# PorousMediaSimulation/openLBMPM

Hardware: AMD Instinct MI355X
Metric: MLUPS (million lattice updates/s) (higher is better)
Workload: dtype f64

## Files before the change

openlbmpm_amd/csrc/rk3dq.h:

```cpp

constexpr int QS = 23;
constexpr unsigned CELLB = QS * 8u;
constexpr int QLINE = 16;
constexpr int SR = 12, SC = 68;
constexpr int SCOMP = SR * SC;
constexpr int SSLOT = 4 * SCOMP;

typedef const unsigned long long __attribute__((address_space(4))) *const_u64_ptr;
__device__ __forceinline__ unsigned long long pstart_of(const RK3Dev &p, int zl) { return ((const_u64_ptr)p.pstart)[zl]; }

struct PlaneAddrQ {
    const char *base;
    unsigned off[3], cnt[3];
};

__device__ __forceinline__ PlaneAddrQ plane_addr_q(const RK3Dev &p, const double *f, int zl)
{
    PlaneAddrQ a;
    const unsigned long long p1 = pstart_of(p, zl), p2 = pstart_of(p, zl + 1);
    const unsigned long long p0 = zl > 0 ? pstart_of(p, zl - 1) : p1, p3 = zl <= p.nzl ? pstart_of(p, zl + 2) : p2;
    a.base = reinterpret_cast<const char *>(f) + (size_t)p0 * CELLB;
    a.cnt[0] = (unsigned)(p1 - p0); a.cnt[1] = (unsigned)(p2 - p1); a.cnt[2] = (unsigned)(p3 - p2);
    a.off[0] = 0u; a.off[1] = a.cnt[0] * CELLB; a.off[2] = a.off[1] + a.cnt[1] * CELLB;
    return a;
}

template <bool ASM>
__device__ __forceinline__ double ldq(const char *uniform_base, unsigned off)
{
    if (!ASM) return ldg(uniform_base, off);
    double v;
    asm volatile("global_load_dwordx2 %0, %1, %2" : "=v"(v) : "v"(off), "s"(uniform_base));
    return v;
}
#define LBMPM_WAIT_VMCNT0 0x0F70

template <bool FIRST, bool UNI, typename Rows, bool ASM = false>
__device__ __forceinline__ void pull_q(const RK3Dev &p, const Rows &rows, int zl, unsigned b, double g[Q], unsigned &own_j)
{
    constexpr int OPP[Q] = LBMPM_D3Q19_OPP;
    const PlaneAddrQ a = plane_addr_q(p, p.fin, zl);
    {
        const RowTab t = rows(zl, 0);
        own_j = t.first + bits_below<UNI>(t.m, b);
    }
    const unsigned own8 = own_j * 8u;
    if (FIRST) {
#pragma unroll
        for (int i = 0; i < Q; ++i) g[i] = ldq<ASM>(a.base, a.off[1] + (unsigned)i * a.cnt[1] * 8u + own8);
        return;
    }
#pragma unroll
    for (int rz = -1; rz <= 1; ++rz)
#pragma unroll
        for (int ry = -1; ry <= 1; ++ry) {
            const RowTab t = rows(zl + rz, ry);
#pragma unroll
            for (int dx = -1; dx <= 1; ++dx) {
                const int i = DIRT[(1 - rz) * 9 + (1 - ry) * 3 + (1 - dx)];
                if (i < 0) continue;
                unsigned off;
                if (i == 0) off = a.off[1] + own8;
                else {
                    unsigned j;
                    bool fl;
                    row_cell<UNI>(t, dx, b, j, fl);
                    const unsigned up = a.off[1 + rz] + (unsigned)i * a.cnt[1 + rz] * 8u + j * 8u;
                    const unsigned back = a.off[1] + (unsigned)OPP[i] * a.cnt[1] * 8u + own8;
                    off = fl ? up : back;
                }
                g[i] = ldq<ASM>(a.base, off);
            }
        }
}

__device__ __forceinline__ unsigned row_index(const RK3Dev &p, int zl, int y, int sg) { return ((unsigned)zl * (unsigned)p.ny + (unsigned)y) * (unsigned)p.nseg + (unsigned)sg; }

struct LdsScal {
    const double *tile;
    int own;
    int slot[3];
    typedef int H;
    __device__ __forceinline__ H own_cell() const { return slot[1] + own; }
    __device__ __forceinline__ H cell(int rz, int ry, int dx, bool fl, unsigned, unsigned, unsigned) const { return fl ? slot[1 + rz] + own + ry * SC + dx : slot[1] + own; }
    __device__ __forceinline__ double comp(H h, int k) const { return tile[h + k * SCOMP]; }
};
struct GlbScal {
    const uint32_t *pur_in;
    int ny, nseg;
    const char *base;
    unsigned soff[3];
    unsigned own_j;
    int zp, sg, y;
    struct H { unsigned off, cst; };
    __device__ __forceinline__ H at(int rz, int ry, int sgs, unsigned j) const
    {
        int s = sg + sgs;
        s = s < 0 ? s + nseg : (s >= nseg ? s - nseg : s);
        H h;
        h.cst = pur_in[((size_t)(zp + rz) * ny + wrapi(y + ry, ny)) * nseg + s];
        h.off = soff[1 + rz] + j * 32u;
        return h;
    }
    __device__ __forceinline__ H own_cell() const { return at(0, 0, 0, own_j); }
    __device__ __forceinline__ H cell(int rz, int ry, int dx, bool fl, unsigned j, unsigned b, unsigned last) const
    {
        if (!fl) return own_cell();
        return at(rz, ry, (dx < 0 && b == 0u) ? -1 : ((dx > 0 && b == last) ? 1 : 0), j);
    }
    __device__ __forceinline__ double comp(H h, int k) const
    {
        if (h.cst) return k == 0 && (h.cst & 1u) ? 1. : 0.;
        return *reinterpret_cast<const double *>(base + h.off + 8u * (unsigned)k);
    }
};
__device__ __forceinline__ GlbScal glb_scal(const RK3Dev &p, const PlaneAddrQ &a, unsigned own_j, int zp, int sg, int y)
{
    GlbScal s{p.pur_in, p.ny, p.nseg, a.base, {0u, 0u, 0u}, own_j, zp, sg, y};
#pragma unroll
    for (int k = 0; k < 3; ++k) s.soff[k] = a.off[k] + (unsigned)Q * a.cnt[k] * 8u;
    return s;
}

struct Sums { double k0, kp, km, a0, ap, am, t0, tp, tm; };

template <int CLS, bool FIRST, bool UNI, typename Rows, typename Scal>
__device__ __forceinline__ void class_sum_one(const RK3Dev &p, const Rows &rows, const Scal &sc, int zp, unsigned b, const double g[Q],
                                              double &ks, double &as, double &ts)
{
#pragma clang fp contract(off)
    constexpr int CX[Q] = LBMPM_D3Q19_CX, CY[Q] = LBMPM_D3Q19_CY, CZ[Q] = LBMPM_D3Q19_CZ;
    constexpr int rz = -CLS;
    ks = 0.; as = 0.; ts = 0.;
    if (CLS == 0) { ks = sc.comp(sc.own_cell(), 0) * g[0]; ts = g[0]; }
#pragma unroll
    for (int ry = -1; ry <= 1; ++ry) {
        RowTab t{};
        if (!FIRST) t = rows(zp + rz, ry);
#pragma unroll
        for (int dx = -1; dx <= 1; ++dx) {
            const int i = DIRT[(1 - rz) * 9 + (1 - ry) * 3 + (1 - dx)];
            if (i <= 0) continue;
            unsigned j = 0;
            bool fl = true;
            typename Scal::H h;
            if (FIRST) h = sc.own_cell();
            else {
                row_cell<UNI>(t, dx, b, j, fl);
                h = sc.cell(rz, ry, dx, fl, j, b, t.last);
            }
            const double k = sc.comp(h, 0);
            double ea = 0.;
            bool any = false;
            if (CX[i] != 0) { const double v = sc.comp(h, 1); ea = CX[i] > 0 ? v : -v; any = true; }
            if (CY[i] != 0) { const double v = sc.comp(h, 2); ea = any ? (CY[i] > 0 ? ea + v : ea - v) : (CY[i] > 0 ? v : -v); any = true; }
            if (CZ[i] != 0) { const double v = sc.comp(h, 3); ea = any ? (CZ[i] > 0 ? ea + v : ea - v) : (CZ[i] > 0 ? v : -v); }
            const double c = i < 7 ? p.rcA : p.rcD;
            const double cs = fl ? c : -c;
            ks = __builtin_fma(k, g[i], ks); as = __builtin_fma(cs, ea, as); ts += g[i];
        }
    }
}

template <bool FIRST, bool UNI, typename Rows, typename Scal>
__device__ __forceinline__ void class_sums(const RK3Dev &p, const Rows &rows, const Scal &sc, int zp, unsigned b, const double g[Q], Sums &S)
{
    class_sum_one<1, FIRST, UNI>(p, rows, sc, zp, b, g, S.kp, S.ap, S.tp);
    class_sum_one<0, FIRST, UNI>(p, rows, sc, zp, b, g, S.k0, S.a0, S.t0);
    class_sum_one<-1, FIRST, UNI>(p, rows, sc, zp, b, g, S.km, S.am, S.tm);
}

template <int CLS, bool FIRST, typename Rows>
__device__ __forceinline__ void pull_class(const RK3Dev &p, const Rows &rows, int zl, unsigned b, unsigned own_j, double g[Q])
{
    constexpr int OPP[Q] = LBMPM_D3Q19_OPP;
    constexpr int rz = -CLS;
    const PlaneAddrQ a = plane_addr_q(p, p.fin, zl);
    const unsigned own8 = own_j * 8u;
    if (CLS == 0) g[0] = ldg(a.base, a.off[1] + own8);
#pragma unroll
    for (int ry = -1; ry <= 1; ++ry) {
        RowTab t{};
        if (!FIRST) t = rows(zl + rz, ry);
#pragma unroll
        for (int dx = -1; dx <= 1; ++dx) {
            const int i = DIRT[(1 - rz) * 9 + (1 - ry) * 3 + (1 - dx)];
            if (i <= 0) continue;
            unsigned j = 0;
            bool fl = true;
            if (!FIRST) row_cell<false>(t, dx, b, j, fl);
            const unsigned up = a.off[1 + rz] + (unsigned)i * a.cnt[1 + rz] * 8u + j * 8u;
            const unsigned back = a.off[1] + (unsigned)OPP[i] * a.cnt[1] * 8u + own8;
            g[i] = ldg(a.base, FIRST ? a.off[1] + (unsigned)i * a.cnt[1] * 8u + own8 : (fl ? up : back));
        }
    }
}

__device__ __forceinline__ void class_sums_pure(const double g[Q], bool red, Sums &S)
{
#pragma clang fp contract(off)
    constexpr int CZ[Q] = LBMPM_D3Q19_CZ;
    S.t0 = g[0]; S.tp = 0.; S.tm = 0.;
#pragma unroll
    for (int rz = -1; rz <= 1; ++rz)
#pragma unroll
        for (int ry = -1; ry <= 1; ++ry)
#pragma unroll
            for (int dx = -1; dx <= 1; ++dx) {
                const int i = DIRT[(1 - rz) * 9 + (1 - ry) * 3 + (1 - dx)];
                if (i <= 0) continue;
                if (CZ[i] == 0) S.t0 += g[i];
                else if (CZ[i] > 0) S.tp += g[i];
                else S.tm += g[i];
            }
    S.k0 = red ? S.t0 : 0.; S.kp = red ? S.tp : 0.; S.km = red ? S.tm : 0.;
    S.a0 = S.ap = S.am = 0.;
}

template <bool WITH_G, int PIN = -1>
__device__ __forceinline__ void bc_q(const RK3Dev &p, int zl, const Sums &S, double *g, double &rR, double &rho)
{
#pragma clang fp contract(off)
    const bool pin = PIN < 0 ? p.inletP != 0 : PIN == 1;
    const int zsg = p.z0 + source_plane(p, zl) - 1;
    const double r0 = S.k0 + S.a0, rp = S.kp + S.ap, rm = S.km + S.am;
    rR = (r0 + rp) + rm;
    rho = (S.t0 + S.tp) + S.tm;
    if (zsg == p.nzg - 2) {
        const double wR = r0 + 2. * rp, wT = S.t0 + 2. * S.tp;
        double J;
        if (pin) {
            rR = p.vzR;
            rho = p.vzR + p.vzB;
            J = wT - rho;
        } else {
            const double dR = wR / (1. + p.vzR), dB = (wT - wR) / (1. + p.vzB);
            rR = dR;
            rho = dR + dB;
            J = dR * p.vzR + dB * p.vzB;
        }
        if (WITH_G) {
            const double Nx = 0.5 * ((g[1] + g[7] + g[9]) - (g[2] + g[8] + g[10]));
            const double Ny = 0.5 * ((g[3] + g[7] + g[10]) - (g[4] + g[8] + g[9]));
            g[6] = g[5] - 1. / 3. * J;
            g[12] = g[11] - 1. / 6. * J + Nx;
            g[13] = g[14] - 1. / 6. * J - Nx;
            g[16] = g[15] - 1. / 6. * J + Ny;
            g[17] = g[18] - 1. / 6. * J - Ny;
        }
    }
    if (zsg == 1) {
        rR = p.rhoOutR;
        rho = p.rhoOutR + p.rhoOutB;
        if (WITH_G) {
            const double J = rho - (S.t0 + 2. * S.tm);
            const double Nx = 0.5 * ((g[1] + g[7] + g[9]) - (g[2] + g[8] + g[10]));
            const double Ny = 0.5 * ((g[3] + g[7] + g[10]) - (g[4] + g[8] + g[9]));
            g[5] = g[6] + 1. / 3. * J;
            g[11] = g[12] + 1. / 6. * J - Nx;
            g[14] = g[13] + 1. / 6. * J + Nx;
            g[15] = g[16] + 1. / 6. * J - Ny;
            g[18] = g[17] + 1. / 6. * J + Ny;
        }
    }
}
__device__ __forceinline__ double phi_q(double rR, double rho) { return (rR - (rho - rR)) / rho; }

template <bool FIRST, bool MRT, bool RAGGED, bool PIN = false>
__global__ __launch_bounds__(512, 1) void rk3dq_fused(RK3Dev p, int tilesX, int tilesY, int rows_per_xcd, int chunk_len, int z_first, int z_last,
                                                       int nchunks1, int z_first2, int z_last2,
                                                       unsigned *slotq)
{
    constexpr int TX = 64, TY = 8;
    using M = March<TX, TY>;
    using TR = TileRows<TY>;
    constexpr int CX[Q] = LBMPM_D3Q19_CX, CY[Q] = LBMPM_D3Q19_CY, CZ[Q] = LBMPM_D3Q19_CZ;
    __shared__ double sphi[M::RING][M::FY][M::FX];
    __shared__ double ssc[4 * SSLOT];
    __shared__ u32x4 srow[TR::SLOTS][TR::ROWS][6];
    __shared__ int sslot[2];
    const int tid = threadIdx.x;
    const int band_slots = (int)(gridDim.x >> 3);
    if (tid == 0 && !slotq) { sslot[0] = (int)(blockIdx.x & 7u); sslot[1] = (int)(blockIdx.x >> 3); }
    if (tid == 0 && slotq) {
        const int here = (int)(__builtin_amdgcn_s_getreg((3 << 11) | 20) & 7u);
        int band = -1, slot = 0;
        for (int k = 0; k < 8 && band < 0; ++k) {
            const int b = (here + k) & 7;
            const int q = (int)atomicAdd(&slotq[b], 1u);
            if (q < band_slots) { band = b; slot = q; }
        }
        sslot[0] = band; sslot[1] = slot;
    }
    __syncthreads();
    const int xcd = sslot[0], slot = sslot[1];
    if (xcd < 0) return;
#ifdef LBMPM_DEV
    const int bid = xcd + 8 * slot;
#endif
    const int tx = slot % tilesX, r = slot / tilesX, ty = xcd * rows_per_xcd + r % rows_per_xcd, chunk = r / rows_per_xcd;
    if (ty >= tilesY) return;
    const int wave = __builtin_amdgcn_readfirstlane(tid >> 6);
#ifdef LBMPM_DEV
    unsigned long long *trace = p.trace && z_last - z_first >= 8 ? p.trace + (size_t)bid * 4 : nullptr;
    if (trace && tid == 0) trace[0] = wall_clock64();
#endif
    int lx, ly, x, y, yo, hlx, hly, hx, hy, xrow, xc, xcol;
    bool own, has_own, has_rim, has_x, row_ok;
    TileRowsU<TY, true, RAGGED> rows_own{{srow, 0, 1}}, rows_rimrow{{srow, 0, 1}}, rows_xrow{{srow, 0, 1}};
    TileRowsU<TY, false, RAGGED> rows_rimcol{{srow, 0, 0}}, rows_xcol{{srow, 0, 0}};
    const int x0 = RAGGED ? seg_x0(tx, p.nx, tilesX) : tx * TX;
    const int tw = RAGGED ? seg_x0(tx + 1, p.nx, tilesX) - x0 : TX;
    const int twl = RAGGED ? (tx > 0 ? x0 - seg_x0(tx - 1, p.nx, tilesX) : p.nx - seg_x0(tilesX - 1, p.nx, tilesX)) : TX;
    auto set_geometry = [&](int t) {
        lx = t % TX; ly = t / TX;
        x = x0 + lx; y = ty * TY + ly;
        own = y < p.ny;
        yo = ring_coord(y, p.ny);
        row_ok = yo >= 0;
        has_own = row_ok && lx < tw;
        hlx = 0; hly = 0; hx = 0; hy = 0;
        has_rim = false;
        if (t < M::NH) {
            bool in_row = true;
            if (t < 2 * TX) { hlx = 1 + t % TX; hly = t < TX ? 0 : M::FY - 1; in_row = t % TX < tw; }
            else { const int k = t - 2 * TX; hlx = k < M::FY ? 0 : tw + 1; hly = k < M::FY ? k : k - M::FY; }
            hx = ring_coord(x0 + hlx - 1, p.nx);
            hy = ring_coord(ty * TY + hly - 1, p.ny);
            has_rim = hx >= 0 && hy >= 0 && in_row;
        }
        xrow = ly >= 3 && ly <= 6 ? (ly < 5 ? ly - 5 : ly + 3) : (lx >> 2) - 2;
        xc = lx & 3; xcol = ly == 7 ? (xc < 2 ? xc - 2 : tw + xc - 2) : lx;
        has_x = (ly >= 3 && ly <= 6) || (ly == 7 && lx < 4 * SR);
        rows_own.t.lrow = ly + 2;
        rows_rimrow.t.lrow = hly + 1;
        rows_rimcol.t.lrow = hly + 1; rows_rimcol.t.k = hlx == 0 ? 0 : 2;
        rows_xrow.t.lrow = xrow + 2;
        rows_xcol.t.lrow = xrow + 2; rows_xcol.t.k = xc < 2 ? 0 : 2;
    };
    set_geometry(tid);
    __shared__ unsigned sgeo[3][TX * TY];
    sgeo[0][tid] = (unsigned)lx | ((unsigned)ly << 6) | ((unsigned)hlx << 9) | ((unsigned)hly << 16) | ((unsigned)(xrow + 2) << 20) | ((unsigned)xc << 24) |
                   ((unsigned)own << 26) | ((unsigned)has_own << 27) | ((unsigned)has_rim << 28) | ((unsigned)has_x << 29) | ((unsigned)row_ok << 30);
    sgeo[1][tid] = ((unsigned)hx & 0xffffu) | ((unsigned)hy << 16);
    sgeo[2][tid] = ((unsigned)yo & 0xffffu) | ((unsigned)(xcol + 2) << 16);
    auto load_geometry = [&](int t) {
        const unsigned w0 = sgeo[0][t], w1 = sgeo[1][t], w2 = sgeo[2][t];
        lx = (int)(w0 & 63u); ly = (int)((w0 >> 6) & 7u);
        x = x0 + lx; y = ty * TY + ly;
        hlx = (int)((w0 >> 9) & 127u); hly = (int)((w0 >> 16) & 15u);
        xrow = (int)((w0 >> 20) & 15u) - 2; xc = (int)((w0 >> 24) & 3u);
        own = (w0 >> 26) & 1u; has_own = (w0 >> 27) & 1u; has_rim = (w0 >> 28) & 1u; has_x = (w0 >> 29) & 1u;
        row_ok = RAGGED ? (w0 >> 30) & 1u : has_own;
        hx = (int)(short)(w1 & 0xffffu); hy = (int)w1 >> 16;
        yo = (int)(short)(w2 & 0xffffu); xcol = (int)(w2 >> 16) - 2;
        rows_own.t.lrow = ly + 2;
        rows_rimrow.t.lrow = hly + 1;
        rows_rimcol.t.lrow = hly + 1; rows_rimcol.t.k = hlx == 0 ? 0 : 2;
        rows_xrow.t.lrow = xrow + 2;
        rows_xcol.t.lrow = xrow + 2; rows_xcol.t.k = xc < 2 ? 0 : 2;
    };
    const int za = chunk < nchunks1 ? z_first + chunk * chunk_len : z_first2 + (chunk - nchunks1) * chunk_len;
    const int zb = min(za + chunk_len - 1, chunk < nchunks1 ? z_last : z_last2);
    const int zl_gb = 1 - p.z0, zl_gt = p.nzg - p.z0;
    auto is_ghost = [&](int zl) { return zl == zl_gb || zl == zl_gt; };
    struct RowRec { u32x4 v; unsigned f0, f1, f2; };
    auto fetch_rows = [&](int zl) -> RowRec {
        RowRec q;
        q.v = u32x4{0u, 0u, 0u, 0u}; q.f0 = 0u; q.f1 = ~0u; q.f2 = ~0u;
        if (tid < TR::ROWS * 6 && zl >= 0 && zl <= p.nzl + 1) {
            const int row = tid / 6, k = tid % 6;
            int yy = (ty * TY - 2 + row) % p.ny;
            if (yy < 0) yy += p.ny;
            int sg = tx - 1 + (k >> 1);
            sg = sg < 0 ? sg + p.nseg : (sg >= p.nseg ? sg - p.nseg : sg);
            const unsigned rr = ((unsigned)zl * (unsigned)p.ny + (unsigned)yy) * (unsigned)p.nseg + (unsigned)sg;
            q.v = (k & 1) ? p.seg2[rr] : p.seg[rr];
            if (k & 1) {
                q.f0 = p.pur_in[rr];
                if (k == 3) {
                    const int sl = tx > 0 ? tx - 1 : p.nseg - 1, sr = tx + 1 < p.nseg ? tx + 1 : 0;
                    q.f1 = p.pur_in[rr - sg + sl]; q.f2 = p.pur_in[rr - sg + sr];
                }
            }
        }
        return q;
    };
    auto put_rows = [&](int zl, const RowRec &q) {
        if (tid < TR::ROWS * 6) {
            u32x4 v = q.v;
            if (tid & 1) { v.z = q.f0; v.w = q.f0 & q.f1 & q.f2; }
            const_cast<u32x4 &>(srow[zl & (TR::SLOTS - 1)][tid / 6][tid % 6]) = v;
        }
    };
    auto row_flag = [&](int zl, int lrow, int k) -> unsigned { return srow[zl & (TR::SLOTS - 1)][lrow][2 * k + 1].z; };
    struct SRec { double2 a, b; bool ok; };
    auto load_s = [&](int zl, unsigned j) -> SRec {
        const unsigned long long p0 = pstart_of(p, zl);
        const unsigned cnt = (unsigned)(pstart_of(p, zl + 1) - p0);
        const char *s = reinterpret_cast<const char *>(p.fin) + (size_t)p0 * CELLB + (size_t)cnt * (Q * 8u) + (size_t)j * 32u;
        SRec v;
        v.a = *reinterpret_cast<const double2 *>(s); v.b = *reinterpret_cast<const double2 *>(s + 16);
        v.ok = true;
        return v;
    };
    auto const_s = [&](unsigned flag) -> SRec {
        SRec v;
        v.a.x = (flag & 1u) ? 1. : 0.; v.a.y = 0.; v.b.x = 0.; v.b.y = 0.; v.ok = true;
        return v;
    };
    auto fetch_s = [&](int zl, SRec &e0, SRec &e1) {
        e0.ok = false; e1.ok = false;
        if (zl < 0 || zl > p.nzl + 1) return;
        {
            const RowTab t = rows_own(zl, 0);
            const unsigned fg = (unsigned)__builtin_amdgcn_readfirstlane((int)row_flag(zl, ly + 2, 1));
            if (bit_of<true>(t.m, (unsigned)lx)) e0 = fg ? const_s(fg) : load_s(zl, t.first + bits_below<true>(t.m, (unsigned)lx));
        }
        if (wave >= 3 && wave <= 6) {
            const RowTab t = rows_xrow(zl, 0);
            const unsigned fg = (unsigned)__builtin_amdgcn_readfirstlane((int)row_flag(zl, xrow + 2, 1));
            if (bit_of<true>(t.m, (unsigned)lx)) e1 = fg ? const_s(fg) : load_s(zl, t.first + bits_below<true>(t.m, (unsigned)lx));
        } else if (wave == 7) {
            if (has_x) {
                const RowTab t = rows_xcol(zl, 0);
                const unsigned fg = row_flag(zl, xrow + 2, xc < 2 ? 0 : 2);
                const unsigned bb = xc < 2 ? (unsigned)(twl - 2) + (unsigned)xc : (unsigned)xc - 2u;
                if (bit_of<false>(t.m, bb)) e1 = fg ? const_s(fg) : load_s(zl, t.first + bits_below<false>(t.m, bb));
            }
        }
    };
    auto put_s = [&](int zl, const SRec &e0, const SRec &e1) {
        double *sl = ssc + (zl & 3) * SSLOT;
        if (e0.ok) {
            double *d = sl + (ly + 2) * SC + lx + 2;
            d[0] = e0.a.x; d[SCOMP] = e0.a.y; d[2 * SCOMP] = e0.b.x; d[3 * SCOMP] = e0.b.y;
        }
        if (wave >= 3 && e1.ok) {
            double *d = sl + (xrow + 2) * SC + xcol + 2;
            d[0] = e1.a.x; d[SCOMP] = e1.a.y; d[2 * SCOMP] = e1.b.x; d[3 * SCOMP] = e1.b.y;
        }
    };
    auto purity = [&](int zp, int row_lo, int row_hi) -> int {
        unsigned c = 3u;
        for (int dz = -1; dz <= 1; ++dz)
            for (int rr = row_lo - 1; rr <= row_hi + 1; ++rr) c &= srow[(zp + dz) & (TR::SLOTS - 1)][rr + 2][3].w;
        return __builtin_amdgcn_readfirstlane((int)c);
    };
    auto lds_scal = [&](int zp, int row, int col) {
        LdsScal s;
        s.tile = ssc; s.own = (row + 2) * SC + col + 2;
        s.slot[0] = ((zp - 1) & 3) * SSLOT; s.slot[1] = (zp & 3) * SSLOT; s.slot[2] = ((zp + 1) & 3) * SSLOT;
        return s;
    };
    {
        RowRec rr[6];
#pragma unroll
        for (int k = 0; k < 6; ++k) rr[k] = fetch_rows(za - 3 + k);
#pragma unroll
        for (int k = 0; k < 6; ++k) put_rows(za - 3 + k, rr[k]);
    }
    RowRec staged = fetch_rows(za + 3);
    __syncthreads();
    {
        SRec e0[3], e1[3];
#pragma unroll
        for (int k = 0; k < 3; ++k) fetch_s(za - 2 + k, e0[k], e1[k]);
#pragma unroll
        for (int k = 0; k < 3; ++k) put_s(za - 2 + k, e0[k], e1[k]);
    }
    bool fluid = false, fl_raw = false;
    bool padz = false, pad_raw = false;
    unsigned jz = 0, j_raw = 0;
    double rR = 1., rho = 2.;
    bool mixed_w = false, mixed_n = false;
    double raw[Q], cur[Q];
#pragma unroll
    for (int i = 0; i < Q; ++i) { raw[i] = 0.; cur[i] = 0.; }
    auto issue = [&](int zl) {
        fl_raw = false; pad_raw = false;
        if (!row_ok || zl < 1 || zl > p.nzl || is_ghost(zl)) return;
        const RowTab t = rows_own(zl, 0);
        fl_raw = bit_of<true>(t.m, (unsigned)lx);
        if (!fl_raw) {
            const unsigned rank = bits_below<true>(~t.m, (unsigned)lx);
            pad_raw = own && rank < t.pad;
            j_raw = t.first + (unsigned)__popcll(t.m) + rank;
            return;
        }
        pull_q<FIRST, true, decltype(rows_own), true>(p, rows_own, zl, (unsigned)lx, raw, j_raw);
    };
    auto pulls_landed = [&]() {
        __builtin_amdgcn_s_waitcnt(LBMPM_WAIT_VMCNT0);
#pragma unroll
        for (int i = 0; i < Q; ++i) asm volatile("" : "+v"(raw[i]));
    };
    __syncthreads();
    issue(za - 1);
    pulls_landed();
#ifdef LBMPM_DEV
    if (trace && tid == 0) { trace[1] = wall_clock64(); trace[3] = ((unsigned long long)(unsigned)za << 32) | (unsigned)zb; }
#endif

#if defined(LBMPM_DEV) && defined(LBMPM_PHASES)
    unsigned long long ph_acc[6] = {0, 0, 0, 0, 0, 0}, ph_t = 0;
#define PH_MARK(k) { const unsigned long long now_ = __builtin_readcyclecounter(); if (z >= za) ph_acc[k] += now_ - ph_t; ph_t = now_; }
#else
#define PH_MARK(k)
#endif
    for (int z = za - 2; z <= zb; ++z) {
        const int zn = z + 1;
#if defined(LBMPM_DEV) && defined(LBMPM_PHASES)
        ph_t = __builtin_readcyclecounter();
#endif
        {
            int t = tid;
            asm volatile("" : "+v"(t));
#ifdef LBMPM_RK3D_GEO_COMPUTE
            set_geometry(t);
#else
            load_geometry(t);
#endif
        }
        const unsigned long long pz0 = pstart_of(p, z > 0 ? z : 0), pz1 = pstart_of(p, z > 0 ? z + 1 : 1);
        put_rows(z + 5, staged);
        SRec e0, e1;
        fetch_s(z + 3, e0, e1);
        const bool halo_n = zn <= p.halo_lo || zn >= p.nzl + 1, ghost_n = !halo_n && is_ghost(zn);
        const bool fill_gb = !halo_n && !ghost_n && zn - 1 == zl_gb && zn - 1 >= 1;
        if (wave < 3) {
            if (has_rim) {
                double ph = p.solidPhi;
                if (halo_n) ph = (p.phi + (size_t)zn * p.plane2)[(size_t)hy * p.pitch + hx];
                else if (ghost_n) { if (zn == zl_gt) ph = sphi[z & (M::RING - 1)][hly][hlx]; }
                else {
                    double g[Q], a, c;
                    unsigned j;
                    Sums S;
                    const int pc = wave < 2 ? purity(zn, hly - 1, hly - 1) : purity(zn, -1, TY);
                    const unsigned hb = RAGGED ? (hlx == 0 ? (unsigned)(twl - 1) : 0u) : (unsigned)(hx & 63);
                    const bool fl = wave < 2 ? bit_of<true>(rows_rimrow(zn, 0).m, (unsigned)lx) : bit_of<false>(rows_rimcol(zn, 0).m, hb);
                    if (pc != 0) {
                        if (fl) {
                            S.t0 = 1.; S.tp = S.tm = 0.; S.k0 = (pc & 1) ? 1. : 0.; S.kp = S.km = S.a0 = S.ap = S.am = 0.;
                            bc_q<false, PIN ? 1 : 0>(p, zn, S, nullptr, a, c);
                            ph = phi_q(a, c);
                        }
                    } else if (wave < 2) {
                        if (fl) {
                            pull_q<FIRST, true>(p, rows_rimrow, zn, (unsigned)lx, g, j);
                            class_sums<FIRST, true>(p, rows_rimrow, lds_scal(zn, hly - 1, hlx - 1), zn, (unsigned)lx, g, S);
                            bc_q<false, PIN ? 1 : 0>(p, zn, S, nullptr, a, c);
                            ph = phi_q(a, c);
                        }
                    } else if (fl) {
                        pull_q<FIRST, false>(p, rows_rimcol, zn, hb, g, j);
                        class_sums<FIRST, false>(p, rows_rimcol, lds_scal(zn, hly - 1, hlx - 1), zn, hb, g, S);
                        bc_q<false, PIN ? 1 : 0>(p, zn, S, nullptr, a, c);
                        ph = phi_q(a, c);
                    }
                }
                sphi[zn & (M::RING - 1)][hly][hlx] = ph;
                if (fill_gb) sphi[(zn - 1) & (M::RING - 1)][hly][hlx] = ph;
            }
        }
        PH_MARK(0)
        double ft[Q];
        const double rRz = rR, rhoz = rho;
        const unsigned jzz = jz;
        const bool mixed_z = mixed_w;
        mixed_n = false;
        const bool fluidn = fl_raw && !halo_n && !ghost_n;
        {
            double rRn = 1., rhon = 2., ph = p.solidPhi;
            if (halo_n) { if (has_own) ph = (p.phi + (size_t)zn * p.plane2)[(size_t)yo * p.pitch + x]; }
            else if (ghost_n) { if (has_own && zn == zl_gt) ph = sphi[z & (M::RING - 1)][ly + 1][lx + 1]; }
            else if (fl_raw) {
                Sums S;
                const int pc = purity(zn, ly, ly);
                mixed_n = pc == 0;
                if (pc != 0) class_sums_pure(raw, (pc & 1) != 0, S);
                else class_sums<FIRST, true>(p, rows_own, lds_scal(zn, ly, lx), zn, (unsigned)lx, raw, S);
                bc_q<true, PIN ? 1 : 0>(p, zn, S, raw, rRn, rhon);
                ph = phi_q(rRn, rhon);
            }
            if (has_own) {
                sphi[zn & (M::RING - 1)][ly + 1][lx + 1] = ph;
                if (fill_gb) sphi[(zn - 1) & (M::RING - 1)][ly + 1][lx + 1] = ph;
            }
#pragma unroll
            for (int i = 0; i < Q; ++i) { ft[i] = cur[i]; cur[i] = raw[i]; }
            rR = rRn; rho = rhon; jz = j_raw; mixed_w = mixed_n;
        }
        const bool padzz = padz;
        padz = pad_raw;
        PH_MARK(1)
        put_s(z + 3, e0, e1);
        __builtin_amdgcn_s_waitcnt(LBMPM_WAIT_VMCNT0);
        PH_MARK(2)
        if (z + 2 <= zb + 1) issue(z + 2);
        else { fl_raw = false; pad_raw = false; }
        staged = fetch_rows(z + 6);
        PH_MARK(3)
        __syncthreads();
        PH_MARK(4)
        const bool live = z >= za && !is_ghost(z);
        const bool active = live && fluid && own;
        if (__ballot(active) == 0ull) {
            pulls_landed();
            if (live && own && lx == 0) p.pur_out[row_index(p, z, y, tx)] = 3u;
        } else if (active) {
            LBMPM_TAKEN;
            double ax = 0., ay = 0., az = 0., dx = 0., dy = 0., dz = 0.;
#pragma unroll
            for (int i = 1; i < Q; ++i) {
                const double ph = sphi[(z + CZ[i]) & (M::RING - 1)][ly + 1 + CY[i]][lx + 1 + CX[i]];
                if (i < 7) {
                    if (CX[i] != 0) ax = CX[i] > 0 ? ax + ph : ax - ph;
                    if (CY[i] != 0) ay = CY[i] > 0 ? ay + ph : ay - ph;
                    if (CZ[i] != 0) az = CZ[i] > 0 ? az + ph : az - ph;
                } else {
                    if (CX[i] != 0) dx = CX[i] > 0 ? dx + ph : dx - ph;
                    if (CY[i] != 0) dy = CY[i] > 0 ? dy + ph : dy - ph;
                    if (CZ[i] != 0) dz = CZ[i] > 0 ? dz + ph : dz - ph;
                }
            }
            const double gx = 3. * wq(1) * ax + 3. * wq(7) * dx, gy = 3. * wq(1) * ay + 3. * wq(7) * dy, gz = 3. * wq(1) * az + 3. * wq(7) * dz;
            if (__builtin_amdgcn_readfirstlane((int)mixed_z))
                collide_store<2, MRT, true>(p, reinterpret_cast<char *>(p.fout) + (size_t)pz0 * CELLB, (unsigned)(pz1 - pz0) * 8u, jzz * 8u, true, ft, rRz,
                                            rhoz - rRz, gx, gy, gz, p.pur_out + row_index(p, z, y, tx));
            else
                collide_store<2, MRT>(p, reinterpret_cast<char *>(p.fout) + (size_t)pz0 * CELLB, (unsigned)(pz1 - pz0) * 8u, jzz * 8u, true, ft, rRz, rhoz - rRz,
                                      gx, gy, gz, p.pur_out + row_index(p, z, y, tx));
        }
        if (live && padzz) {
            char *pl = reinterpret_cast<char *>(p.fout) + (size_t)pz0 * CELLB;
            const unsigned stride = (unsigned)(pz1 - pz0) * 8u;
#pragma unroll
            for (int i = 0; i < Q; ++i) stg(pl + (size_t)i * stride, jzz * 8u, 0.);
        }
#pragma unroll
        for (int i = 0; i < Q; ++i) asm volatile("" : "+v"(raw[i]));
        fluid = fluidn;
        PH_MARK(5)
    }
#undef PH_MARK
#if defined(LBMPM_DEV) && defined(LBMPM_PHASES)
    if (p.trace && (tid & 63) == 0 && bid < 4096) {
        unsigned long long *o = p.trace + (1u << 18) + ((size_t)bid * 8 + (size_t)wave) * 8;
        for (int k = 0; k < 6; ++k) o[k] = ph_acc[k];
        o[6] = (unsigned long long)(zb - za + 1);
    }
#endif
#ifdef LBMPM_DEV
    if (trace && tid == 0) trace[2] = wall_clock64();
#endif
}

__global__ __launch_bounds__(BX3 *BY3) void rk3dq_init_rest(RK3Dev p, const double *rho_r, const double *rho_b, double *f, uint32_t *pur)
{
    const int sg = blockIdx.x, x = LBMPM_SEG_LANE_X(p, sg, (int)threadIdx.x), y = blockIdx.y * BY3 + threadIdx.y, zl = blockIdx.z + 1;
    if (y >= p.ny) return;
    const bool fluid = x >= 0 && (p.flags[(size_t)zl * p.plane2 + (size_t)y * p.pitch + x] & 1);
    double a = 0., b = 0.;
    if (fluid) {
        const GlobalRows rows{p, sg, y};
        const RowTab t = rows(zl, 0);
        const unsigned j = t.first + bits_below<false>(t.m, threadIdx.x);
        const size_t sd = ((size_t)(zl - 1) * p.ny + y) * p.nx + x;
        a = rho_r[sd]; b = rho_b[sd];
        const unsigned long long p0 = pstart_of(p, zl);
        const size_t cnt = (size_t)(pstart_of(p, zl + 1) - p0);
        double *pl = f + (size_t)p0 * QS;
        for (int i = 0; i < Q; ++i) pl[(size_t)i * cnt + j] = wq(i) * (a + b);
        double *s = pl + (size_t)Q * cnt + (size_t)j * 4;
        s[0] = a / (a + b); s[1] = 0.; s[2] = 0.; s[3] = 0.;
    }
    const unsigned code = (__ballot(fluid && b != 0.) == 0ull ? 1u : 0u) | (__ballot(fluid && a != 0.) == 0ull ? 2u : 0u);
    if (threadIdx.x == 0) pur[row_index(p, zl, y, sg)] = code;
}

__global__ __launch_bounds__(BX3 *BY3) void rk3dq_phase_field(RK3Dev p, int zl0)
{
    const int sg = blockIdx.x, x = LBMPM_SEG_LANE_X(p, sg, (int)threadIdx.x), y = blockIdx.y * BY3 + threadIdx.y, zl = blockIdx.z + zl0;
    if (y >= p.ny || x < 0) return;
    const size_t idx = (size_t)zl * p.plane2 + (size_t)y * p.pitch + x;
    if (!(p.flags[idx] & 1)) return;
    const int zs = source_plane_x(p, zl);
    const unsigned b = threadIdx.x;
    double g[Q], rR, rho;
    unsigned j;
    Sums S;
    const GlobalRows rows{p, sg, y};
    if (p.first) {
        pull_q<true, false>(p, rows, zs, b, g, j);
        class_sums<true, false>(p, rows, glb_scal(p, plane_addr_q(p, p.fin, zs), j, zs, sg, y), zs, b, g, S);
    } else {
        pull_q<false, false>(p, rows, zs, b, g, j);
        class_sums<false, false>(p, rows, glb_scal(p, plane_addr_q(p, p.fin, zs), j, zs, sg, y), zs, b, g, S);
    }
    bc_q<true>(p, p.conv && p.z0 + zl - 1 <= 2 ? zs : zl, S, g, rR, rho);
    p.phi[idx] = phi_q(rR, rho);
    if (p.diag) {
        constexpr int CX[Q] = LBMPM_D3Q19_CX, CY[Q] = LBMPM_D3Q19_CY, CZ[Q] = LBMPM_D3Q19_CZ;
        double mx = 0., my = 0., mz = 0.;
#pragma unroll
        for (int i = 0; i < Q; ++i) { mx += (double)CX[i] * g[i]; my += (double)CY[i] * g[i]; mz += (double)CZ[i] * g[i]; }
        p.diag[idx] = rR; p.diag[p.vol + idx] = rho - rR;
        p.diag[2 * p.vol + idx] = mx / rho; p.diag[3 * p.vol + idx] = my / rho; p.diag[4 * p.vol + idx] = mz / rho;
    }
}

__global__ __launch_bounds__(256) void rk3dq_conv_phi(RK3Dev p, int zs)
{
    const size_t k = (size_t)blockIdx.x * blockDim.x + threadIdx.x;
    if (k >= p.plane2 || !(p.flags[(size_t)zs * p.plane2 + k] & 1)) return;
    const double v = p.phi[(size_t)zs * p.plane2 + k];
    for (int zl = zs - 3; zl < zs; ++zl) p.phi[(size_t)zl * p.plane2 + k] = v;
}

template <bool FIRST, bool MRT>
__global__ __launch_bounds__(BX3 *BY3) void rk3dq_conv_collide(RK3Dev p, int zs)
{
    constexpr int CX[Q] = LBMPM_D3Q19_CX, CY[Q] = LBMPM_D3Q19_CY, CZ[Q] = LBMPM_D3Q19_CZ;
    const int sg = blockIdx.x, x = LBMPM_SEG_LANE_X(p, sg, (int)threadIdx.x), y = blockIdx.y * BY3 + threadIdx.y, zl = zs - 1 - (int)blockIdx.z;
    if (y >= p.ny) return;
    const bool fluid = x >= 0 && (p.flags[(size_t)zl * p.plane2 + (size_t)y * p.pitch + x] & 1);
    if (__ballot(fluid) == 0ull) {
        if (threadIdx.x == 0) p.pur_out[row_index(p, zl, y, sg)] = 3u;
        return;
    }
    if (!fluid) return;
    const GlobalRows rows{p, sg, y};
    const unsigned b = threadIdx.x;
    double g[Q], rR, rho;
    unsigned js;
    Sums S;
    pull_q<FIRST, false>(p, rows, zs, b, g, js);
    class_sums<FIRST, false>(p, rows, glb_scal(p, plane_addr_q(p, p.fin, zs), js, zs, sg, y), zs, b, g, S);
    bc_q<true>(p, zs, S, g, rR, rho);
    double gx = 0., gy = 0., gz = 0.;
    const int xs[3] = {wrapi(x - 1, p.nx), x, wrapi(x + 1, p.nx)}, ys[3] = {wrapi(y - 1, p.ny), y, wrapi(y + 1, p.ny)};
#pragma unroll
    for (int i = 1; i < Q; ++i) {
        const double ph = p.phi[(size_t)(zl + CZ[i]) * p.plane2 + (size_t)ys[1 + CY[i]] * p.pitch + xs[1 + CX[i]]];
        gx += 3. * wq(i) * (double)CX[i] * ph;
        gy += 3. * wq(i) * (double)CY[i] * ph;
        gz += 3. * wq(i) * (double)CZ[i] * ph;
    }
    const RowTab t = rows(zl, 0);
    const unsigned j = t.first + bits_below<false>(t.m, b);
    const unsigned long long p0 = pstart_of(p, zl);
    const unsigned cnt = (unsigned)(pstart_of(p, zl + 1) - p0);
    collide_store<2, MRT>(p, reinterpret_cast<char *>(p.fout) + (size_t)p0 * CELLB, cnt * 8u, j * 8u, true, g, rR, rho - rR, gx, gy, gz,
                          p.pur_out + row_index(p, zl, y, sg));
}

constexpr int FACE_DOUBLES = 13;
__device__ constexpr int FACE_UP[5] = {5, 11, 14, 15, 18}, FACE_DN[5] = {6, 12, 13, 16, 17};

__global__ __launch_bounds__(BX3 *BY3) void rk3dq_face_pack(RK3Dev p, double *send_up, double *send_dn, int has_below, int has_above)
{
    const int sg = blockIdx.x, x = LBMPM_SEG_LANE_X(p, sg, (int)threadIdx.x), y = blockIdx.y * BY3 + threadIdx.y, face = blockIdx.z;
    if ((face == 0 && !has_above) || (face == 1 && !has_below) || y >= p.ny) return;
    const int zf = face == 0 ? p.nzl : 1;
    double *msg = face == 0 ? send_up : send_dn;
    const unsigned long long p0 = pstart_of(p, zf);
    const size_t cnt = (size_t)(pstart_of(p, zf + 1) - p0);
    const unsigned flag = p.pur_in[row_index(p, zf, y, sg)];
    if (threadIdx.x == 0) reinterpret_cast<uint32_t *>(msg + FACE_DOUBLES * cnt)[y * p.nseg + sg] = flag;
    if (x < 0 || !(p.flags[(size_t)zf * p.plane2 + (size_t)y * p.pitch + x] & 1)) return;
    const GlobalRows rows{p, sg, y};
    const unsigned b = threadIdx.x;
    const RowTab t = rows(zf, 0);
    const unsigned j = t.first + bits_below<false>(t.m, b);
    const double *pl = p.fin + (size_t)p0 * QS;
    for (int k = 0; k < 5; ++k) msg[(size_t)k * cnt + j] = pl[(size_t)(face == 0 ? FACE_UP[k] : FACE_DN[k]) * cnt + j];
    const double *s = pl + (size_t)Q * cnt + (size_t)j * 4;
    double *ms = msg + 5 * cnt + (size_t)j * 4;
    if (flag) { ms[0] = (flag & 1u) ? 1. : 0.; ms[1] = 0.; ms[2] = 0.; ms[3] = 0.; }
    else { ms[0] = s[0]; ms[1] = s[1]; ms[2] = s[2]; ms[3] = s[3]; }
    double g[Q], k0, a0, t0, kx, ax, tx;
    const GlbScal sc = glb_scal(p, plane_addr_q(p, p.fin, zf), j, zf, sg, y);
    double *mp = msg + 9 * cnt + (size_t)j * 4;
    if (p.first) {
        double km, am, tm;
        pull_class<0, true>(p, rows, zf, b, j, g); pull_class<1, true>(p, rows, zf, b, j, g); pull_class<-1, true>(p, rows, zf, b, j, g);
        class_sum_one<0, true, false>(p, rows, sc, zf, b, g, k0, a0, t0);
        class_sum_one<1, true, false>(p, rows, sc, zf, b, g, kx, ax, tx);
        class_sum_one<-1, true, false>(p, rows, sc, zf, b, g, km, am, tm);
        mp[0] = (k0 + a0) + (kx + ax); mp[1] = km + am; mp[2] = t0 + tx; mp[3] = tm;
        return;
    }
    pull_class<0, false>(p, rows, zf, b, j, g);
    class_sum_one<0, false, false>(p, rows, sc, zf, b, g, k0, a0, t0);
    if (face == 0) { pull_class<1, false>(p, rows, zf, b, j, g); class_sum_one<1, false, false>(p, rows, sc, zf, b, g, kx, ax, tx); }
    else { pull_class<-1, false>(p, rows, zf, b, j, g); class_sum_one<-1, false, false>(p, rows, sc, zf, b, g, kx, ax, tx); }
    mp[0] = k0 + a0; mp[1] = kx + ax; mp[2] = t0; mp[3] = tx;
}

__global__ __launch_bounds__(BX3 *BY3) void rk3dq_face_unpack(RK3Dev p, double *f, uint32_t *pur, const double *recv_below, const double *recv_above,
                                                              int has_below, int has_above)
{
    const int sg = blockIdx.x, x = LBMPM_SEG_LANE_X(p, sg, (int)threadIdx.x), y = blockIdx.y * BY3 + threadIdx.y, face = blockIdx.z;
    if ((face == 0 && !has_below) || (face == 1 && !has_above) || y >= p.ny) return;
    const int zh = face == 0 ? 0 : p.nzl + 1;
    const double *msg = face == 0 ? recv_below : recv_above;
    const unsigned long long p0 = pstart_of(p, zh);
    const size_t cnt = (size_t)(pstart_of(p, zh + 1) - p0);
    if (threadIdx.x == 0) pur[row_index(p, zh, y, sg)] = reinterpret_cast<const uint32_t *>(msg + FACE_DOUBLES * cnt)[y * p.nseg + sg];
    if (x < 0 || !(p.flags[(size_t)zh * p.plane2 + (size_t)y * p.pitch + x] & 1)) return;
    const GlobalRows rows{p, sg, y};
    const RowTab t = rows(zh, 0);
    const unsigned j = t.first + bits_below<false>(t.m, threadIdx.x);
    double *pl = f + (size_t)p0 * QS;
    for (int k = 0; k < 5; ++k) pl[(size_t)(face == 0 ? FACE_UP[k] : FACE_DN[k]) * cnt + j] = msg[(size_t)k * cnt + j];
    double *s = pl + (size_t)Q * cnt + (size_t)j * 4;
    const double *ms = msg + 5 * cnt + (size_t)j * 4;
    s[0] = ms[0]; s[1] = ms[1]; s[2] = ms[2]; s[3] = ms[3];
}

__global__ __launch_bounds__(BX3 *BY3) void rk3dq_halo_phi(RK3Dev p, const double *recv_below, const double *recv_above, int has_below, int has_above)
{
    const int sg = blockIdx.x, x = LBMPM_SEG_LANE_X(p, sg, (int)threadIdx.x), y = blockIdx.y * BY3 + threadIdx.y, face = blockIdx.z;
    if ((face == 0 && !has_below) || (face == 1 && !has_above) || y >= p.ny || x < 0) return;
    const int zh = face == 0 ? 0 : p.nzl + 1;
    const size_t idx = (size_t)zh * p.plane2 + (size_t)y * p.pitch + x;
    if (!(p.flags[idx] & 1)) return;
    const double *msg = face == 0 ? recv_below : recv_above;
    const size_t cnt = (size_t)(pstart_of(p, zh + 1) - pstart_of(p, zh));
    const GlobalRows rows{p, sg, y};
    const unsigned b = threadIdx.x;
    const RowTab t = rows(zh, 0);
    const unsigned j = t.first + bits_below<false>(t.m, b);
    const double *mp = msg + 9 * cnt + (size_t)j * 4;
    Sums S;
    S.a0 = S.ap = S.am = 0.;
    if (p.first) {
        S.k0 = mp[0]; S.kp = 0.; S.km = mp[1]; S.t0 = mp[2]; S.tp = 0.; S.tm = mp[3];
    } else {
        double g[Q];
        const GlbScal sc = glb_scal(p, plane_addr_q(p, p.fin, zh), j, zh, sg, y);
        S.k0 = mp[0]; S.t0 = mp[2];
        if (face == 0) {
            S.kp = mp[1]; S.tp = mp[3];
            pull_class<-1, false>(p, rows, zh, b, j, g);
            class_sum_one<-1, false, false>(p, rows, sc, zh, b, g, S.km, S.am, S.tm);
        } else {
            S.km = mp[1]; S.tm = mp[3];
            pull_class<1, false>(p, rows, zh, b, j, g);
            class_sum_one<1, false, false>(p, rows, sc, zh, b, g, S.kp, S.ap, S.tp);
        }
    }
    double rR, rho;
    bc_q<false>(p, zh, S, nullptr, rR, rho);
    p.phi[idx] = phi_q(rR, rho);
}

__global__ __launch_bounds__(BX3 *BY3) void rk3dq_debug_plane(RK3Dev p, const double *f, int zl, int comp, double *out)
{
    const int sg = blockIdx.x, x = LBMPM_SEG_LANE_X(p, sg, (int)threadIdx.x), y = blockIdx.y * BY3 + threadIdx.y;
    if (y >= p.ny || x < 0) return;
    double v = 0.;
    if (p.flags[(size_t)zl * p.plane2 + (size_t)y * p.pitch + x] & 1) {
        const GlobalRows rows{p, sg, y};
        const RowTab t = rows(zl, 0);
        const unsigned j = t.first + bits_below<false>(t.m, threadIdx.x);
        const unsigned long long p0 = pstart_of(p, zl);
        const size_t cnt = (size_t)(pstart_of(p, zl + 1) - p0);
        const double *pl = f + (size_t)p0 * QS;
        v = comp < Q ? pl[(size_t)comp * cnt + j] : pl[(size_t)Q * cnt + (size_t)j * 4 + (comp - Q)];
    }
    out[(size_t)y * p.nx + x] = v;
}
```

Measured before the change: 13880.

## Precompute per-cell compact index map in LDS for neighbour pulls

Adds a shared-memory ring of per-cell compact indices (with pad and none markers) built once per plane from the row bitmask tables. The pull step then reads the 19 neighbour indices from this map instead of recomputing popcount/bit ranks for every direction per cell. This trades repeated ALU and row-table decoding for extra LDS footprint, extra map-building work each plane, and an added barrier, which may reduce occupancy or add sync cost.

```diff
diff --git a/openlbmpm_amd/csrc/rk3dq.h b/openlbmpm_amd/csrc/rk3dq.h
--- a/openlbmpm_amd/csrc/rk3dq.h
+++ b/openlbmpm_amd/csrc/rk3dq.h
@@ -72,6 +72,52 @@
                 g[i] = ldq<ASM>(a.base, off);
             }
         }
+}
+
+constexpr unsigned CELLMAP_PAD = 0x80000000u, CELLMAP_NONE = 0xFFFFFFFFu;
+
+template <int FX>
+__device__ __forceinline__ void read_map(const unsigned *const mq[3], unsigned m[Q])
+{
+    m[0] = mq[1][FX + 1];
+#pragma unroll
+    for (int rz = -1; rz <= 1; ++rz)
+#pragma unroll
+        for (int ry = -1; ry <= 1; ++ry)
+#pragma unroll
+            for (int dx = -1; dx <= 1; ++dx) {
+                const int i = DIRT[(1 - rz) * 9 + (1 - ry) * 3 + (1 - dx)];
+                if (i > 0) m[i] = mq[1 + rz][(1 + ry) * FX + 1 + dx];
+            }
+}
+template <bool FIRST>
+__device__ __forceinline__ void pull_q_map(const RK3Dev &p, const unsigned m[Q], int zl, unsigned own_j, double g[Q])
+{
+    constexpr int OPP[Q] = LBMPM_D3Q19_OPP;
+    const PlaneAddrQ a = plane_addr_q(p, p.fin, zl);
+    const unsigned own8 = own_j * 8u;
+    if (FIRST) {
+#pragma unroll
+        for (int i = 0; i < Q; ++i) g[i] = ldq<true>(a.base, a.off[1] + (unsigned)i * a.cnt[1] * 8u + own8);
+        return;
+    }
+#pragma unroll
+    for (int rz = -1; rz <= 1; ++rz)
+#pragma unroll
+        for (int ry = -1; ry <= 1; ++ry)
+#pragma unroll
+            for (int dx = -1; dx <= 1; ++dx) {
+                const int i = DIRT[(1 - rz) * 9 + (1 - ry) * 3 + (1 - dx)];
+                if (i < 0) continue;
+                unsigned off;
+                if (i == 0) off = a.off[1] + own8;
+                else {
+                    const unsigned up = a.off[1 + rz] + (unsigned)i * a.cnt[1 + rz] * 8u + m[i] * 8u;
+                    const unsigned back = a.off[1] + (unsigned)OPP[i] * a.cnt[1] * 8u + own8;
+                    off = (int)m[i] >= 0 ? up : back;
+                }
+                g[i] = ldq<true>(a.base, off);
+            }
 }
 
 __device__ __forceinline__ unsigned row_index(const RK3Dev &p, int zl, int y, int sg) { return ((unsigned)zl * (unsigned)p.ny + (unsigned)y) * (unsigned)p.nseg + (unsigned)sg; }
@@ -278,6 +324,7 @@
     __shared__ double sphi[M::RING][M::FY][M::FX];
     __shared__ double ssc[4 * SSLOT];
     __shared__ u32x4 srow[TR::SLOTS][TR::ROWS][6];
+    __shared__ unsigned sj[M::RING][M::FY][M::FX];
     __shared__ int sslot[2];
     const int tid = threadIdx.x;
     const int band_slots = (int)(gridDim.x >> 3);
@@ -393,6 +440,28 @@
             const_cast<u32x4 &>(srow[zl & (TR::SLOTS - 1)][tid / 6][tid % 6]) = v;
         }
     };
+    auto put_map_row = [&](int zl, const RowTab &t, int mrow, bool pads) {
+        unsigned *d = sj[zl & (M::RING - 1)][mrow];
+        unsigned v = t.first + bits_below<true>(t.m, (unsigned)lx);
+        if (!bit_of<true>(t.m, (unsigned)lx)) {
+            v = CELLMAP_NONE;
+            if (pads) {
+                const unsigned rank = bits_below<true>(~t.m, (unsigned)lx);
+                if (rank < t.pad) v = CELLMAP_PAD | (t.first + (unsigned)__popcll(t.m) + rank);
+            }
+        }
+        d[!RAGGED || lx < tw ? lx + 1 : lx + 2] = v;
+        if (lx == 0) d[0] = t.lbit ? t.jl : CELLMAP_NONE;
+        if (lx == tw - 1) d[tw + 1] = t.rbit ? t.jr : CELLMAP_NONE;
+    };
+    auto put_map = [&](int zl) {
+        if (wave >= 4) return;
+        const TileRowsU<TY, true, RAGGED> ra{{srow, wave + 2, 1}}, rb{{srow, wave + 6, 1}}, rc{{srow, wave == 0 ? 1 : TY + 2, 1}};
+        const RowTab ta = ra(zl, 0), tb = rb(zl, 0);
+        put_map_row(zl, ta, wave + 1, true);
+        put_map_row(zl, tb, wave + 5, true);
+        if (wave == 0 || wave == 3) put_map_row(zl, rc(zl, 0), wave == 0 ? 0 : TY + 1, false);
+    };
     auto row_flag = [&](int zl, int lrow, int k) -> unsigned { return srow[zl & (TR::SLOTS - 1)][lrow][2 * k + 1].z; };
     struct SRec { double2 a, b; bool ok; };
     auto load_s = [&](int zl, unsigned j) -> SRec {
@@ -462,6 +531,7 @@
     }
     RowRec staged = fetch_rows(za + 3);
     __syncthreads();
+    for (int k = 0; k < 4; ++k) put_map(za - 2 + k);
     {
         SRec e0[3], e1[3];
 #pragma unroll
@@ -480,15 +550,17 @@
     auto issue = [&](int zl) {
         fl_raw = false; pad_raw = false;
         if (!row_ok || zl < 1 || zl > p.nzl || is_ghost(zl)) return;
-        const RowTab t = rows_own(zl, 0);
-        fl_raw = bit_of<true>(t.m, (unsigned)lx);
+        const unsigned *const mq[3] = {&sj[(zl - 1) & (M::RING - 1)][ly][lx], &sj[zl & (M::RING - 1)][ly][lx], &sj[(zl + 1) & (M::RING - 1)][ly][lx]};
+        unsigned m[Q];
+        read_map<M::FX>(mq, m);
+        const unsigned mo = !RAGGED || lx < tw ? m[0] : mq[1][M::FX + 2];
+        fl_raw = (int)mo >= 0;
+        j_raw = mo & ~CELLMAP_PAD;
         if (!fl_raw) {
-            const unsigned rank = bits_below<true>(~t.m, (unsigned)lx);
-            pad_raw = own && rank < t.pad;
-            j_raw = t.first + (unsigned)__popcll(t.m) + rank;
+            pad_raw = own && mo != CELLMAP_NONE;
             return;
         }
-        pull_q<FIRST, true, decltype(rows_own), true>(p, rows_own, zl, (unsigned)lx, raw, j_raw);
+        pull_q_map<FIRST>(p, m, zl, j_raw, raw);
     };
     auto pulls_landed = [&]() {
         __builtin_amdgcn_s_waitcnt(LBMPM_WAIT_VMCNT0);
@@ -497,6 +569,7 @@
     };
     __syncthreads();
     issue(za - 1);
+    __syncthreads();
     pulls_landed();
 #ifdef LBMPM_DEV
     if (trace && tid == 0) { trace[1] = wall_clock64(); trace[3] = ((unsigned long long)(unsigned)za << 32) | (unsigned)zb; }
@@ -524,6 +597,7 @@
         }
         const unsigned long long pz0 = pstart_of(p, z > 0 ? z : 0), pz1 = pstart_of(p, z > 0 ? z + 1 : 1);
         put_rows(z + 5, staged);
+        put_map(z + 4);
         SRec e0, e1;
         fetch_s(z + 3, e0, e1);
         const bool halo_n = zn <= p.halo_lo || zn >= p.nzl + 1, ghost_n = !halo_n && is_ghost(zn);
```

Measured after the change: 13540. -2.5%, worse.
